# thilinarmtb/lsbench

Measured on AMD Instinct MI355X. Metric: cg_solves_per_sec, higher is better.
Workload: dtype f64

## Files before the change

### lsbench_amd/csrc/hip_kernels.hip

```cpp
#include "hip_kcommon.h"

__device__ __forceinline__ void spmv_publish(double *__restrict__ partials, double dot,
                                             double *sred, const lsb_ar_tail &tail) {
  if (!partials)
    return;
  double d[1] = {dot};
  wg_sum<1>(d, sred);
  if (tail.counter)
    ar_tail(partials, d[0], tail);
  else if (threadIdx.x == 0)
    partials[blockIdx.x] = d[0];
}

enum { SP_PREFETCH = 1, SP_NT = 2 };

template <int FLAGS, class T>
__device__ __forceinline__ T stream_load(const T *p) {
  if (FLAGS & SP_NT)
    return __builtin_nontemporal_load(p);
  return *p;
}

#define LSB_ISSUE_BLOCK(kk)                                                    \
  do {                                                                         \
// ... 722 lines not shown
      }
    } else if (row + 1 < n) {
      const sell_d2v o = {a0, a1};
      *(sell_d2v *)(y + row) = o;
      if (xdot) {
        dot = fma(a0, xd.x, dot);
        dot = fma(a1, xd.y, dot);
      }
    } else if (row < n) {
      y[row] = a0;
      if (xdot)
        dot = fma(a0, xd.x, dot);
    }
  }
#pragma unroll
  for (int k = 0; k < DEFER_DEPTH; k++)
    TMPL_UNPARK_SLOT(k);
#undef TMPL_UNPARK
#undef TMPL_UNPARK_SLOT
  if (stopped)
    return;
  spmv_publish(partials, dot, sred, tail);
}

template <int NF> struct col_ops {
  sell_d2u lo[NF > 1 ? NF - 1 : 1], hi[NF > 1 ? NF - 1 : 1];
  double edge;
  sell_d2v xd;
};
template <int NF> struct col_tmpl {
  int bc, bl[NF > 1 ? NF - 1 : 1], bh[NF > 1 ? NF - 1 : 1];
  double k0, kl[NF > 1 ? NF - 1 : 1], kc, kh[NF > 1 ? NF - 1 : 1], kL;
};
template <int NF, int DOT>
__device__ __forceinline__ void col_issue(col_ops<NF> &o, sell_d2u &cnext, const col_tmpl<NF> &T, const double *__restrict__ x,
                                          const double *__restrict__ xdot, long long gu, unsigned lrow, long long D,
                                          unsigned xlen, unsigned lane, bool with_next) {
  if (with_next)
    cnext = *(const sell_d2u *)(x + (gu + T.bc + D) + 2 * lane);
#pragma unroll
  for (int k = 0; k < NF - 1; k++) {
    o.lo[k] = *(const sell_d2u *)(x + (gu + T.bl[k]) + 2 * lane);
    o.hi[k] = *(const sell_d2u *)(x + (gu + T.bh[k]) + 2 * lane);
  }
  long long el = gu + T.bc - 1, er = gu + T.bc + (long long)LSB_SELL_ROWS;
  el = el < 0 ? 0 : el, er = er >= (long long)xlen ? (long long)xlen - 1 : er;
  o.edge = x[lane < 32u ? el : er];
  if (DOT == 2)
    o.xd = *(const sell_d2v *)(xdot + lrow + 2 * lane);
}
template <int NF, int DOT>
__device__ __forceinline__ void col_compute(const col_ops<NF> &o, const sell_d2u &cm, const sell_d2u &c, const sell_d2u &cp,
                                            const col_tmpl<NF> &T, double vm0, double vm1, double vp0, double vp1,
                                            unsigned lane, double &a0, double &a1, double &dot) {
  double up = lane_above(c.y), dn = lane_below(c.x);
  if (lane == 0)
    up = o.edge;
  if (lane == 63)
    dn = o.edge;
  a0 = fma(T.k0, cm.x, 0.0), a1 = fma(T.k0, cm.y, 0.0);
#pragma unroll
  for (int k = 0; k < NF - 1; k++)
    a0 = fma(T.kl[k], o.lo[k].x, a0), a1 = fma(T.kl[k], o.lo[k].y, a1);
  a0 = fma(vm0, vm0 != 0.0 ? up : 0.0, a0), a1 = fma(vm1, vm1 != 0.0 ? c.x : 0.0, a1);
  a0 = fma(T.kc, c.x, a0), a1 = fma(T.kc, c.y, a1);
  a0 = fma(vp0, vp0 != 0.0 ? c.y : 0.0, a0), a1 = fma(vp1, vp1 != 0.0 ? dn : 0.0, a1);
#pragma unroll
  for (int k = 0; k < NF - 1; k++)
    a0 = fma(T.kh[k], o.hi[k].x, a0), a1 = fma(T.kh[k], o.hi[k].y, a1);
  a0 = fma(T.kL, cp.x, a0), a1 = fma(T.kL, cp.y, a1);
  if (DOT == 1)
    dot = fma(a0, c.x, dot), dot = fma(a1, c.y, dot);
  else if (DOT == 2)
    dot = fma(a0, o.xd.x, dot), dot = fma(a1, o.xd.y, dot);
}

#define LSB_COL_HEAD 16
__device__ __forceinline__ bool col_walks_down(const unsigned *__restrict__ plan, unsigned dofs, unsigned it) {
  return dofs && ((plan[dofs + (it >> 5)] >> (it & 31u)) & 1u);
}
template <int NF, int DOT>
__global__ __launch_bounds__(WG, DOT == 2 ? 5 : 6) void k_spmv_tmpl_col(
    const unsigned *__restrict__ plan, unsigned period, unsigned n, unsigned row_begin, unsigned xlen,
    const unsigned *__restrict__ sptr, const unsigned long long *__restrict__ mask,
    const lsb_sell_tmpl *__restrict__ td, const int *__restrict__ sbase, const void *__restrict__ vals, int f32,
    const double *__restrict__ vconst, const double *__restrict__ x, double *__restrict__ y,
    const double *__restrict__ xdot, double *__restrict__ partials, const lsb_pcg_state *__restrict__ st,
    const lsb_ar_tail tail) {
  static_assert(NF >= 1 && NF <= 2, "one or two far slots per side");
  __shared__ double sred[4];
  const unsigned tid = threadIdx.x, lane = tid & 63u, wave = tid >> 6;
  const unsigned gx = gridDim.x / NXCD, xcd = blockIdx.x % NXCD, slot = blockIdx.x / NXCD;
  const unsigned i0 = plan[xcd], i1 = plan[xcd + 1];
  const u4v *__restrict__ items = (const u4v *)(plan + LSB_COL_HEAD);
  const unsigned dofs = plan[LSB_TMPL_COL_DOWN];
  const int stopped = st ? st->status : 0;
  const unsigned P = period * LSB_SELL_ROWS;
  double dot = 0.0;
  for (unsigned g = slot; i0 + 4 * g < i1; g += gx) {
    const unsigned it = __builtin_amdgcn_readfirstlane(i0 + 4 * g + wave);
    if (it >= i1)
      continue;
    const u4v rec = items[it];
    const unsigned s = __builtin_amdgcn_readfirstlane(rec.x), Kw = __builtin_amdgcn_readfirstlane(rec.y);
    const unsigned K = Kw & ~LSB_TMPL_COL_LOCKSTEP;
    const bool lockstep = (Kw & LSB_TMPL_COL_LOCKSTEP) != 0;
    if (K >= 2) {
      const unsigned t = __builtin_amdgcn_readfirstlane(rec.z), mb = __builtin_amdgcn_readfirstlane(rec.w);
      const lsb_sell_tmpl *T = td + t;
      col_tmpl<NF> C;
      C.bc = T->base[NF + 1];
      C.k0 = T->cst[0], C.kc = T->cst[NF + 1], C.kL = T->cst[2 * NF + 2];
// ... 75 lines not shown
          const sell_d2u v = *(const sell_d2u *)(x + (grow + r.x));
          a0 = fma(k, v.x, a0), a1 = fma(k, v.y, a1);
        } else {
          double v0, v1;
          if (f32) {
            const vt2<float>::type v = *((const vt2<float>::type *)((const float *)vals + (size_t)r.z * LSB_SELL_ROWS) + lane);
            v0 = (double)v.x, v1 = (double)v.y;
          } else {
            const sell_d2v v = *((const sell_d2v *)((const double *)vals + (size_t)r.z * LSB_SELL_ROWS) + lane);
            v0 = v.x, v1 = v.y;
          }
          const bool p0 = v0 != 0.0, p1 = v1 != 0.0;
          const double t0 = x[p0 ? grow + r.x : 0], t1 = x[p1 ? grow + 1 + r.x : 0];
          a0 = fma(v0, p0 ? t0 : 0.0, a0), a1 = fma(v1, p1 ? t1 : 0.0, a1);
        }
      }
      if (row + 1 < n) {
        const sell_d2v o = {a0, a1};
        *(sell_d2v *)(y + row) = o;
        if (DOT)
          dot = fma(a0, xd.x, dot), dot = fma(a1, xd.y, dot);
      } else if (row < n) {
        y[row] = a0;
        if (DOT)
          dot = fma(a0, xd.x, dot);
      }
    }
  }
  if (stopped)
    return;
  spmv_publish(partials, dot, sred, tail);
}

template <int NF> struct colp_c {
  sell_d2u rn, pn;
  sell_d2v xn, sn;
  double re, pe;
};
template <int NF> struct colp_m {
  sell_d2u rlo[NF > 1 ? NF - 1 : 1], plo[NF > 1 ? NF - 1 : 1], rhi[NF > 1 ? NF - 1 : 1], phi[NF > 1 ? NF - 1 : 1];
};
struct colp_out {
  sell_d2v q, x, p;
};
template <int NF, bool WITH_X, int NT>
__device__ __forceinline__ void colp_issue_c(colp_c<NF> &o, const col_tmpl<NF> &T, const double *__restrict__ r,
                                             const double *__restrict__ pold, const double *__restrict__ x,
                                             const double *pstale, long long gu, long long D, unsigned xlen,
                                             unsigned lane) {
  const long long ga = gu + T.bc + D;
  o.rn = *(const sell_d2u *)(r + ga + 2 * lane);
  o.pn = *(const sell_d2u *)(pold + ga + 2 * lane);
  if (WITH_X) {
    if (NT & 1) {
      o.xn = __builtin_nontemporal_load((const sell_d2v *)(x + (gu + D) + 2 * lane));
      o.sn = __builtin_nontemporal_load((const sell_d2v *)(pstale + (gu + D) + 2 * lane));
    } else {
      o.xn = *(const sell_d2v *)(x + (gu + D) + 2 * lane);
      o.sn = *(const sell_d2v *)(pstale + (gu + D) + 2 * lane);
    }
  }
  long long el = gu + T.bc - 1, er = gu + T.bc + (long long)LSB_SELL_ROWS;
  el = el < 0 ? 0 : el, er = er >= (long long)xlen ? (long long)xlen - 1 : er;
  const long long e = lane < 32u ? el : er;
  o.re = r[e], o.pe = pold[e];
}
template <int NF>
__device__ __forceinline__ void colp_issue_m(colp_m<NF> &o, const col_tmpl<NF> &T, const double *__restrict__ r,
                                             const double *__restrict__ pold, long long gu, unsigned lane) {
#pragma unroll
  for (int k = 0; k < NF - 1; k++) {
    o.rlo[k] = *(const sell_d2u *)(r + (gu + T.bl[k]) + 2 * lane);
    o.plo[k] = *(const sell_d2u *)(pold + (gu + T.bl[k]) + 2 * lane);
    o.rhi[k] = *(const sell_d2u *)(r + (gu + T.bh[k]) + 2 * lane);
    o.phi[k] = *(const sell_d2u *)(pold + (gu + T.bh[k]) + 2 * lane);
  }
}
template <int NF, bool OWNED, bool XUPD>
__device__ __forceinline__ void colp_compute(const colp_c<NF> &o, const colp_m<NF> &m, const sell_d2u &pb,
                                             const sell_d2u &p0, sell_d2u &pp, bool down, const col_tmpl<NF> &T, double vm0,
                                             double vm1, double vp0, double vp1, double beta, double alpha, double alpha2,
                                             double dc, unsigned lane, colp_out &out, double &dot) {
  pp.x = pnew_of(dc, o.rn.x, beta, o.pn.x), pp.y = pnew_of(dc, o.rn.y, beta, o.pn.y);
  if (OWNED) {
    if (XUPD) {
      out.x.x = (o.xn.x + alpha2 * o.sn.x) + alpha * o.pn.x, out.x.y = (o.xn.y + alpha2 * o.sn.y) + alpha * o.pn.y;
    }
    out.p.x = pp.x, out.p.y = pp.y;
  }
  const double edge = pnew_of(dc, o.re, beta, o.pe);
  double up = lane_above(p0.y), dn = lane_below(p0.x);
  if (lane == 0)
    up = edge;
  if (lane == 63)
    dn = edge;
  const sell_d2u &pm = down ? pp : pb, &pu = down ? pb : pp;
  double a0 = fma(T.k0, pm.x, 0.0), a1 = fma(T.k0, pm.y, 0.0);
#pragma unroll
  for (int k = 0; k < NF - 1; k++) {
    const double l0 = pnew_of(dc, m.rlo[k].x, beta, m.plo[k].x), l1 = pnew_of(dc, m.rlo[k].y, beta, m.plo[k].y);
    a0 = fma(T.kl[k], l0, a0), a1 = fma(T.kl[k], l1, a1);
  }
  a0 = fma(vm0, vm0 != 0.0 ? up : 0.0, a0), a1 = fma(vm1, vm1 != 0.0 ? p0.x : 0.0, a1);
  a0 = fma(T.kc, p0.x, a0), a1 = fma(T.kc, p0.y, a1);
  a0 = fma(vp0, vp0 != 0.0 ? p0.y : 0.0, a0), a1 = fma(vp1, vp1 != 0.0 ? dn : 0.0, a1);
#pragma unroll
  for (int k = 0; k < NF - 1; k++) {
    const double h0 = pnew_of(dc, m.rhi[k].x, beta, m.phi[k].x), h1 = pnew_of(dc, m.rhi[k].y, beta, m.phi[k].y);
// ... 20 lines not shown
  for (unsigned j = 0; j < len; j++) {
    const i4v rec = ((const i4v *)sbase)[q0 + j];
    if (rec.z < 0) {
      const double k = vconst[q0 + j];
      const sell_d2u rv = *(const sell_d2u *)(r + ((int)row + rec.x)), pv = *(const sell_d2u *)(pold + ((int)row + rec.x));
      a0 = fma(k, pnew_of(dc, rv.x, beta, pv.x), a0), a1 = fma(k, pnew_of(dc, rv.y, beta, pv.y), a1);
    } else {
      const sell_d2v v = *((const sell_d2v *)(vals + (size_t)rec.z * LSB_SELL_ROWS) + lane);
      const bool p0 = v.x != 0.0, p1 = v.y != 0.0;
      const int c0 = p0 ? (int)row + rec.x : 0, c1 = p1 ? (int)row + 1 + rec.x : 0;
      const double t0 = pnew_of(dc, r[c0], beta, pold[c0]), t1 = pnew_of(dc, r[c1], beta, pold[c1]);
      a0 = fma(v.x, p0 ? t0 : 0.0, a0), a1 = fma(v.y, p1 ? t1 : 0.0, a1);
    }
  }
  const double n0 = pnew_of(dc, r0, beta, o0), n1 = pnew_of(dc, r1, beta, o1);
  if (l0) {
    pnew[row] = n0;
    if (xupd)
      x[row] = (x0 + alpha2 * s0) + alpha * o0;
    if (q)
      q[row] = a0;
    dot = fma(a0, n0, dot);
  }
  if (l1) {
    pnew[row + 1] = n1;
    if (xupd)
      x[row + 1] = (x1 + alpha2 * s1) + alpha * o1;
    if (q)
      q[row + 1] = a1;
    dot = fma(a1, n1, dot);
  }
}

#define COLP_ST(PTR, V, BIT)                                                                   \
  do {                                                                                         \
    if (NT & (BIT))                                                                            \
      __builtin_nontemporal_store((V), (sell_d2v *)(PTR));                                     \
    else                                                                                       \
      *(sell_d2v *)(PTR) = (V);                                                                \
  } while (0)
#define COLP_STORE(OUT, LROW, WITH_Q, WITH_XP)                                                 \
  do {                                                                                         \
    if (WITH_Q)                                                                                \
      COLP_ST(q + (LROW) + 2 * lane, (OUT).q, 2);                                              \
    if (WITH_XP) {                                                                             \
      if (XUPD)                                                                                \
        COLP_ST(x + ((LROW) + Du) + 2 * lane, (OUT).x, 1);                                     \
      COLP_ST(pnew + ((LROW) + Du) + 2 * lane, (OUT).p, 2);                                    \
    }                                                                                          \
  } while (0)

template <int NF, int NT, bool XUPD>
__global__ __launch_bounds__(WG, NF == 2 ? 3 : 5) void k_pcg_col_px(
    const unsigned *__restrict__ plan, unsigned period, unsigned n, const unsigned *__restrict__ sptr,
    const unsigned long long *__restrict__ mask, const lsb_sell_tmpl *__restrict__ td, const int *__restrict__ sbase,
    const double *__restrict__ vals, const double *__restrict__ vconst, const double *__restrict__ r,
    const double *__restrict__ pold, double *pnew, double *__restrict__ x, double dc,
    double *__restrict__ partials, lsb_pcg_state *__restrict__ st, int parity,
    const double *__restrict__ parts2, unsigned nparts2) {
  static_assert(NF >= 1 && NF <= 2, "one or two far slots per side");
  __shared__ double sred[8];
  double *const q = nullptr;
  const unsigned tid = threadIdx.x, lane = tid & 63u, wave = tid >> 6;
  const unsigned gx = gridDim.x / NXCD, xcd = blockIdx.x % NXCD, slot = blockIdx.x / NXCD;
  const int stopped = st->status;
  const double rz_old = st->rz[parity], thresh2 = st->thresh2, alpha = st->alpha[0], alpha2 = st->alpha[1];
  const unsigned i0 = plan[xcd], i1 = plan[xcd + 1];
  double v[2];
  wg_sum_partials<2>(parts2, nparts2, v, sred);
  if (stopped)
    return;
  const double rz_new = v[0], rr = v[1];
  const bool conv = rr <= thresh2;
  if (blockIdx.x == 0 && threadIdx.x == 0) {
    const int it = st->iters + 1;
    st->iters = it;
    st->rr = rr;
    st->rz[parity ^ 1] = rz_new;
    if (conv)
      st->status = LSB_STATUS_CONVERGED;
    else {
      if (XUPD)
        st->xpend = 0;
      if (it >= st->maxit)
        st->pad = 1;
    }
  }
  if (conv)
    return;
  const double beta = rz_new / rz_old;
  const u4v *__restrict__ items = (const u4v *)(plan + LSB_COL_HEAD);
  const unsigned dofs = plan[LSB_TMPL_COL_DOWN];
  const unsigned P = period * LSB_SELL_ROWS;
  double dot = 0.0;
  for (unsigned g = slot; i0 + 4 * g < i1; g += gx) {
    const unsigned it = __builtin_amdgcn_readfirstlane(i0 + 4 * g + wave);
    if (it >= i1)
      continue;
    const u4v rec = items[it];
    const unsigned s = __builtin_amdgcn_readfirstlane(rec.x);
    const unsigned K = __builtin_amdgcn_readfirstlane(rec.y) & ~LSB_TMPL_COL_LOCKSTEP;
    if (K >= 3) {
      const unsigned t = __builtin_amdgcn_readfirstlane(rec.z), mb = __builtin_amdgcn_readfirstlane(rec.w);
      const lsb_sell_tmpl *T = td + t;
      col_tmpl<NF> C;
      C.bc = T->base[NF + 1];
      C.k0 = T->cst[0], C.kc = T->cst[NF + 1], C.kL = T->cst[2 * NF + 2];
#pragma unroll
      for (int k = 0; k < NF - 1; k++) {
        C.bl[k] = T->base[1 + k], C.bh[k] = T->base[NF + 3 + k];
        C.kl[k] = T->cst[1 + k], C.kh[k] = T->cst[NF + 3 + k];
      }
      const int side_k[2] = {T->kidx[NF], T->kidx[NF + 2]}, side_kd[2] = {T->kind[NF], T->kind[NF + 2]};
      const bool down = col_walks_down(plan, dofs, it);
      const unsigned s0 = down ? s + (K - 1) * period : s;
      const long long D = down ? -(long long)P : (long long)P;
      const unsigned Du = (unsigned)D;
      long long gu = (long long)s0 * LSB_SELL_ROWS;
      unsigned lrow = s0 * LSB_SELL_ROWS;
      const long long gc = gu + C.bc;
      const sell_d2u rb = *(const sell_d2u *)(r + (gc - D) + 2 * lane);
      const sell_d2u pb = *(const sell_d2u *)(pold + (gc - D) + 2 * lane);
      const sell_d2u r0 = *(const sell_d2u *)(r + gc + 2 * lane), o0 = *(const sell_d2u *)(pold + gc + 2 * lane);
      sell_d2v x0 = {0.0, 0.0}, s0v = {0.0, 0.0};
      if (XUPD)
        x0 = *(const sell_d2v *)(x + lrow + 2 * lane), s0v = *(const sell_d2v *)(pnew + lrow + 2 * lane);
      colp_c<NF> c0, c1;
      colp_m<NF> m0, m1, m2;
      colp_issue_c<NF, XUPD, NT>(c0, C, r, pold, x, pnew, gu, D, n, lane);
      colp_issue_m<NF>(m0, C, r, pold, gu, lane);
      colp_issue_m<NF>(m1, C, r, pold, gu + D, lane);
      unsigned long long mk[2][2] = {{0ull, 0ull}, {0ull, 0ull}};
#pragma unroll
      for (int side = 0; side < 2; side++)
        if (side_k[side] >= 0 && side_kd[side] == 2) {
          const unsigned long long *mp = mask + 2 * ((size_t)mb + (unsigned)side_k[side]);
          mk[side][0] = mp[0], mk[side][1] = mp[1];
        }
      double vm0 = T->cst[NF], vm1 = vm0, vp0 = T->cst[NF + 2], vp1 = vp0;
      if (side_k[0] >= 0 || side_k[1] >= 0)
        tmpl_side_values(T, NF, 0u, lane, side_k, side_kd, mk, vals, 0, vm0, vm1, vp0, vp1);
      sell_d2u pm, p0, pp;
      pm.x = pnew_of(dc, rb.x, beta, pb.x), pm.y = pnew_of(dc, rb.y, beta, pb.y);
      p0.x = pnew_of(dc, r0.x, beta, o0.x), p0.y = pnew_of(dc, r0.y, beta, o0.y);
      colp_out res;
      res.x.x = (x0.x + alpha2 * s0v.x) + alpha * o0.x, res.x.y = (x0.y + alpha2 * s0v.y) + alpha * o0.y;
      res.p.x = p0.x, res.p.y = p0.y;
      res.q = res.p;
      COLP_STORE(res, lrow - Du, false, true);
      for (unsigned k = 0; k + 2 < K; k++) {
        colp_issue_c<NF, XUPD, NT>(c1, C, r, pold, x, pnew, gu + D, D, n, lane);
        colp_issue_m<NF>(m2, C, r, pold, gu + 2 * D, lane);
        colp_compute<NF, true, XUPD>(c0, m0, pm, p0, pp, down, C, vm0, vm1, vp0, vp1, beta, alpha, alpha2, dc, lane, res, dot);
        COLP_STORE(res, lrow, false, true);
        pm = p0, p0 = pp, c0 = c1, m0 = m1, m1 = m2;
        gu += D, lrow += Du;
      }
      colp_issue_c<NF, false, NT>(c1, C, r, pold, x, pnew, gu + D, D, n, lane);
      colp_compute<NF, true, XUPD>(c0, m0, pm, p0, pp, down, C, vm0, vm1, vp0, vp1, beta, alpha, alpha2, dc, lane, res, dot);
      COLP_STORE(res, lrow, false, true);
      pm = p0, p0 = pp, c0 = c1, m0 = m1;
      gu += D, lrow += Du;
      colp_compute<NF, false, XUPD>(c0, m0, pm, p0, pp, down, C, vm0, vm1, vp0, vp1, beta, alpha, alpha2, dc, lane, res, dot);
      COLP_STORE(res, lrow, false, false);
    } else {
      for (unsigned k = 0; k < K; k++)
        colp_single(s + k * period, n, lane, sptr, sbase, vals, vconst, r, pold, pnew, x, nullptr, beta, alpha, alpha2,
                    XUPD, dc, dot);
    }
  }
  if (partials) {
    double d[1] = {dot};
    wg_sum<1>(d, sred);
    if (threadIdx.x == 0)
      partials[blockIdx.x] = d[0];
  }
}
#undef COLP_STORE
#undef COLP_ST

template <int NF>
__global__ __launch_bounds__(WG, 5) void k_pcg_col_r(
    const unsigned *__restrict__ plan, unsigned period, unsigned n, const unsigned *__restrict__ sptr,
    const unsigned long long *__restrict__ mask, const lsb_sell_tmpl *__restrict__ td, const int *__restrict__ sbase,
    const double *__restrict__ vals, const double *__restrict__ vconst, const double *__restrict__ p,
    double *__restrict__ r, double dc, lsb_pcg_state *__restrict__ st, int parity, int pbuf, int xtwo,
    const double *__restrict__ pq_parts, unsigned npq, double *__restrict__ partials2) {
  static_assert(NF >= 1 && NF <= 2, "one or two far slots per side");
  __shared__ double sred[8];
  const unsigned tid = threadIdx.x, lane = tid & 63u, wave = tid >> 6;
  const unsigned gx = gridDim.x / NXCD, xcd = blockIdx.x % NXCD, slot = blockIdx.x / NXCD;
  const int stopped = st->status, pad = st->pad;
  const double rz = st->rz[parity];
  const unsigned i0 = plan[xcd], i1 = plan[xcd + 1];
  double pqv[1];
  wg_sum_partials<1>(pq_parts, npq, pqv, sred);
  if (stopped)
    return;
  if (pad) {
    if (blockIdx.x == 0 && threadIdx.x == 0)
      st->status = LSB_STATUS_MAXIT;
    return;
  }
  const double pq = pqv[0];
  if (!(pq != 0.0) || !isfinite(pq)) {
    if (blockIdx.x == 0 && threadIdx.x == 0)
      st->status = LSB_STATUS_BREAKDOWN;
    return;
  }
  const double alpha = rz / pq;
  if (blockIdx.x == 0 && threadIdx.x == 0) {
    st->pq = pq, st->alpha[1] = st->alpha[0], st->alpha[0] = alpha, st->xpend = (xtwo ? 3 : 1) + pbuf;
  }
  const u4v *__restrict__ items = (const u4v *)(plan + LSB_COL_HEAD);
  const unsigned dofs = plan[LSB_TMPL_COL_DOWN];
  const unsigned P = period * LSB_SELL_ROWS;
  double acc[2] = {0.0, 0.0}, nodot = 0.0;
#define COLR_FINISH(A0, A1, RV, LROW)                                                          \
  do {                                                                                         \
    sell_d2v rn_;                                                                              \
    rn_.x = (RV).x - alpha * (A0), rn_.y = (RV).y - alpha * (A1);                              \
    *(sell_d2v *)(r + (LROW) + 2 * lane) = rn_;                                                \
    acc[0] += rn_.x * (dc * rn_.x);                                                            \
    acc[0] += rn_.y * (dc * rn_.y);                                                            \
    acc[1] += rn_.x * rn_.x;                                                                   \
    acc[1] += rn_.y * rn_.y;                                                                   \
  } while (0)
  for (unsigned g = slot; i0 + 4 * g < i1; g += gx) {
    const unsigned it = __builtin_amdgcn_readfirstlane(i0 + 4 * g + wave);
    if (it >= i1)
      continue;
    const u4v rec = items[it];
    const unsigned s = __builtin_amdgcn_readfirstlane(rec.x);
    const unsigned K = __builtin_amdgcn_readfirstlane(rec.y) & ~LSB_TMPL_COL_LOCKSTEP;
    if (K >= 3) {
      const unsigned t = __builtin_amdgcn_readfirstlane(rec.z), mb = __builtin_amdgcn_readfirstlane(rec.w);
      const lsb_sell_tmpl *T = td + t;
      col_tmpl<NF> C;
      C.bc = T->base[NF + 1];
      C.k0 = T->cst[0], C.kc = T->cst[NF + 1], C.kL = T->cst[2 * NF + 2];
#pragma unroll
      for (int k = 0; k < NF - 1; k++) {
        C.bl[k] = T->base[1 + k], C.bh[k] = T->base[NF + 3 + k];
        C.kl[k] = T->cst[1 + k], C.kh[k] = T->cst[NF + 3 + k];
      }
      const int side_k[2] = {T->kidx[NF], T->kidx[NF + 2]}, side_kd[2] = {T->kind[NF], T->kind[NF + 2]};
      const bool down = col_walks_down(plan, dofs, it);
      const unsigned s0 = down ? s + (K - 1) * period : s;
      const long long D = down ? -(long long)P : (long long)P;
      const unsigned Du = (unsigned)D;
      long long gu = (long long)s0 * LSB_SELL_ROWS;
      unsigned lrow = s0 * LSB_SELL_ROWS;
      col_ops<NF> cur, nxt;
      sell_d2u cb = *(const sell_d2u *)(p + (gu + C.bc - D) + 2 * lane);
      sell_d2u c0 = *(const sell_d2u *)(p + (gu + C.bc) + 2 * lane);
      sell_d2u ca, cn;
      col_issue<NF, 2>(cur, ca, C, p, r, gu, lrow, D, n, lane, true);
      unsigned long long mk[2][2] = {{0ull, 0ull}, {0ull, 0ull}};
#pragma unroll
      for (int side = 0; side < 2; side++)
        if (side_k[side] >= 0 && side_kd[side] == 2) {
          const unsigned long long *mp = mask + 2 * ((size_t)mb + (unsigned)side_k[side]);
          mk[side][0] = mp[0], mk[side][1] = mp[1];
        }
      double vm0 = T->cst[NF], vm1 = vm0, vp0 = T->cst[NF + 2], vp1 = vp0;
      if (side_k[0] >= 0 || side_k[1] >= 0)
        tmpl_side_values(T, NF, 0u, lane, side_k, side_kd, mk, vals, 0, vm0, vm1, vp0, vp1);
      for (unsigned k = 0; k + 1 < K; k++) {
        col_issue<NF, 2>(nxt, cn, C, p, r, gu + D, lrow + Du, D, n, lane, true);
        double a0, a1;
        col_compute<NF, 0>(cur, down ? ca : cb, c0, down ? cb : ca, C, vm0, vm1, vp0, vp1, lane, a0, a1, nodot);
        COLR_FINISH(a0, a1, cur.xd, lrow);
        cb = c0, c0 = ca, ca = cn, cur = nxt;
        gu += D, lrow += Du;
      }
      double a0, a1;
      col_compute<NF, 0>(cur, down ? ca : cb, c0, down ? cb : ca, C, vm0, vm1, vp0, vp1, lane, a0, a1, nodot);
      COLR_FINISH(a0, a1, cur.xd, lrow);
    } else {
      for (unsigned k = 0; k < K; k++) {
        const unsigned sl = s + k * period, row = sl * LSB_SELL_ROWS + 2 * lane;
        const unsigned q0 = sptr[sl] / LSB_SELL_ROWS, len = (sptr[sl + 1] - sptr[sl]) / LSB_SELL_ROWS;
        const bool l0 = row < n, l1 = row + 1 < n;
        const double r0 = l0 ? r[row] : 0.0, r1 = l1 ? r[row + 1] : 0.0;
        double a0 = 0.0, a1 = 0.0;
        for (unsigned j = 0; j < len; j++) {
          const i4v rec2 = ((const i4v *)sbase)[q0 + j];
          if (rec2.z < 0) {
            const double kk = vconst[q0 + j];
            const sell_d2u pv = *(const sell_d2u *)(p + ((int)row + rec2.x));
            a0 = fma(kk, pv.x, a0), a1 = fma(kk, pv.y, a1);
          } else {
            const sell_d2v v = *((const sell_d2v *)(vals + (size_t)rec2.z * LSB_SELL_ROWS) + lane);
            const bool p0 = v.x != 0.0, p1 = v.y != 0.0;
            const double t0 = p[p0 ? (int)row + rec2.x : 0], t1 = p[p1 ? (int)row + 1 + rec2.x : 0];
            a0 = fma(v.x, p0 ? t0 : 0.0, a0), a1 = fma(v.y, p1 ? t1 : 0.0, a1);
          }
        }
        if (l0) {
          const double rn0 = r0 - alpha * a0;
          r[row] = rn0;
          acc[0] += rn0 * (dc * rn0), acc[1] += rn0 * rn0;
        }
        if (l1) {
          const double rn1 = r1 - alpha * a1;
          r[row + 1] = rn1;
          acc[0] += rn1 * (dc * rn1), acc[1] += rn1 * rn1;
        }
      }
    }
  }
#undef COLR_FINISH
  wg_sum<2>(acc, sred);
  if (threadIdx.x == 0) {
    partials2[2 * blockIdx.x + 0] = acc[0];
    partials2[2 * blockIdx.x + 1] = acc[1];
  }
}


__device__ __forceinline__ unsigned bin_pad(unsigned i) { return i + (i >> 3); }

template <int FLAGS, int BIN_U>
__global__ __launch_bounds__(WG) void k_spmv_binned(
    const unsigned *__restrict__ chunk_begin, unsigned nchunk, const unsigned *__restrict__ rows,
    const unsigned *__restrict__ cols, const double *__restrict__ vals,
    const double *__restrict__ x, double *__restrict__ y, const lsb_pcg_state *__restrict__ st) {
  constexpr unsigned CHUNK = BIN_U * WG;
  __shared__ double sprod[CHUNK + CHUNK / 8 + 8];
  __shared__ unsigned skey[CHUNK + CHUNK / 8 + 8];
  __shared__ double swv[4];
  __shared__ int swf[4];
  __shared__ double sred[4];
  const unsigned tid = threadIdx.x, lane = tid & 63u, wave = tid >> 6;
  const unsigned per = gridDim.x / NXCD;
  const unsigned w = (blockIdx.x % NXCD) * per + blockIdx.x / NXCD;
  if (w >= nchunk)
    return;
  const unsigned e0 = chunk_begin[w], cnt = chunk_begin[w + 1] - e0;
  unsigned r[BIN_U], c[BIN_U];
  double v[BIN_U];
  if (cnt <= CHUNK) {
#pragma unroll
// ... 375 lines not shown
```

### lsbench_amd/csrc/lsb_operator.c

```c
#include "lsb_impl.h"
#include <string.h>
#ifdef _OPENMP
#include <omp.h>
#else
static inline int omp_get_max_threads(void) { return 1; }
#endif

static struct csr *csr_alloc(unsigned nrows, unsigned long long nnz) {
  if (nnz > 0xFFFFFFFFull)
    errx(EXIT_FAILURE, "CSR with %llu non-zeros does not fit 32-bit offsets "
                       "(reference layout, src/lsbench-impl.h:22-26)", nnz);
  struct csr *S = lsb_calloc(struct csr, 1);
  S->nrows = nrows, S->base = 0;
  S->offs = lsb_calloc(unsigned, (size_t)nrows + 1);
  S->cols = lsb_calloc(unsigned, (size_t)nnz);
  S->vals = lsb_calloc(double, (size_t)nnz);
  if (!S->offs || !S->cols || !S->vals)
    errx(EXIT_FAILURE, "out of host memory for a %u-row / %llu-nnz CSR", nrows, nnz);
  return S;
}

void lsb_csr_free(struct csr *A) {
  if (!A)
    return;
// ... 1422 lines not shown
    CC_FAIL(13, "walk directions on z-groups of %u cells, %u items per XCD and turn", period, LSB_TMPL_COL_TURN(T->nfar));
  seen = (unsigned char *)calloc((size_t)ns + 1, 1);
  if (!seen)
    CC_FAIL(4, "out of memory");
  const unsigned nplanes = (ns + period - 1) / period, ngroups = (nplanes + C->kmax - 1) / C->kmax;
  for (unsigned i = 0; i < C->nitem; i++) {
    const unsigned *it = C->item + 4 * (size_t)i;
    const unsigned s = it[0], run = it[1] & ~LSB_TMPL_COL_LOCKSTEP;
    if (it[1] & LSB_TMPL_COL_LOCKSTEP) {
      unsigned xk = 0;
      while (xk + 1 < LSB_COL_XCDS && C->xbeg[xk + 1] <= i)
        xk++;
      const unsigned g0 = C->xbeg[xk] + (i - C->xbeg[xk]) / 4 * 4;
      if (g0 + 4 > C->xbeg[xk + 1])
        CC_FAIL(12, "item %u: lockstep in a turn of fewer than four items", i);
      for (unsigned w = 0; w < 4; w++)
        if (C->item[4 * (size_t)(g0 + w) + 1] != it[1] || run < 2)
          CC_FAIL(12, "item %u: lockstep, but item %u of its turn has another length", i, g0 + w);
    }
    if (run < 1 || run > C->kmax || s < C->s_lo || (unsigned long long)s + (unsigned long long)(run - 1) * period >= C->s_hi)
      CC_FAIL(5, "item %u: %u slices from slice %u, every %u, of [%u, %u)", i, run, s, period, C->s_lo, C->s_hi);
    for (unsigned k = 0; k < run; k++) {
      const unsigned sk = s + k * period;
      if (seen[sk]++)
        CC_FAIL(6, "item %u: slice %u is in two items", i, sk);
      if (run >= 2 && (!col_member(T, sk, period) || !col_same(T, s, sk)))
        CC_FAIL(7, "item %u: slice %u does not continue the column of slice %u", i, sk, s);
    }
    if (run >= 2 && C->centre0 && T->t[T->tid[s]].base[T->nfar + 1] != 0)
      CC_FAIL(10, "item %u: centre base %d in a plan that says 0", i, T->t[T->tid[s]].base[T->nfar + 1]);
    if (run >= 2 && (it[2] != T->tid[s] || it[3] != T->vbase[2 * (size_t)s + 1]))
      CC_FAIL(8, "item %u: template %u / first mask %u, its first slice has %u / %u", i, it[2], it[3], T->tid[s],
              T->vbase[2 * (size_t)s + 1]);
    if (C->down) {
      const unsigned zg = (unsigned)(((unsigned long long)(s / period + 1) * ngroups - 1) / nplanes);
      if (((C->down[i / 32] >> (i % 32)) & 1u) != ((zg & 1u) && run >= 3))
        CC_FAIL(13, "item %u: %u slices walk %s in z-group %u", i, run, ((zg & 1u) && run >= 3) ? "upward" : "downward", zg);
    }
  }
  for (unsigned s = C->s_lo; s < C->s_hi; s++)
    if (!seen[s])
      CC_FAIL(9, "slice %u is in no item", s);
  free(seen);
  return 0;
#undef CC_FAIL
}

void lsb_tmpl_cols_free(struct lsb_tmpl_cols *C) {
  if (!C)
    return;
  free(C->item), free(C->down), free(C);
}

void lsb_sell_tmpls_free(struct lsb_sell_tmpls *T) {
  if (!T)
    return;
  free(T->tid), free(T->vbase), free(T->mask), free(T->t), free(T);
}

void lsb_sell_vc_free(struct lsb_sell_vc *V) {
  if (!V)
    return;
  free(V->slots), free(V->vconst), free(V->vals), free(V);
}

void lsb_sell_free(struct lsb_sell *S) {
// ... 5 lines not shown
```

Measured before the change: 1.085.

## Prefetch next column item's header and first loads during current item tail

The column-walk PCG kernels (k_pcg_col_p and k_pcg_col_r) now load the next work item's plan record, template constants and first-slice operands while the current item's last slices are still being computed. The first item's loads are also issued before the partial-sum reduction. This hides the load latency at item boundaries. The side-value computation is simplified to a mask-only path, and a host-side plan check is added that rejects templates where that simplification would be wrong. Several loads and stores also get wave-uniform base pointers through readfirstlane casts into the global address space, to allow scalar addressing. The cost is higher register pressure from carrying the next item's state, which could hurt occupancy under the existing launch bounds.

After: 1.098, median of 6. About the same (+1.1%).

```diff
diff --git a/lsbench_amd/csrc/hip_kernels.hip b/lsbench_amd/csrc/hip_kernels.hip
--- a/lsbench_amd/csrc/hip_kernels.hip
+++ b/lsbench_amd/csrc/hip_kernels.hip
@@ -778,17 +778,21 @@
   int bc, bl[NF > 1 ? NF - 1 : 1], bh[NF > 1 ? NF - 1 : 1];
   double k0, kl[NF > 1 ? NF - 1 : 1], kc, kh[NF > 1 ? NF - 1 : 1], kL;
 };
-template <int NF, int DOT>
+template <int NF, int DOT, int PART = 3>
 __device__ __forceinline__ void col_issue(col_ops<NF> &o, sell_d2u &cnext, const col_tmpl<NF> &T, const double *__restrict__ x,
                                           const double *__restrict__ xdot, long long gu, unsigned lrow, long long D,
                                           unsigned xlen, unsigned lane, bool with_next) {
-  if (with_next)
+  if ((PART & 1) && with_next)
     cnext = *(const sell_d2u *)(x + (gu + T.bc + D) + 2 * lane);
-#pragma unroll
-  for (int k = 0; k < NF - 1; k++) {
-    o.lo[k] = *(const sell_d2u *)(x + (gu + T.bl[k]) + 2 * lane);
-    o.hi[k] = *(const sell_d2u *)(x + (gu + T.bh[k]) + 2 * lane);
-  }
+  if (PART & 2) {
+#pragma unroll
+    for (int k = 0; k < NF - 1; k++) {
+      o.lo[k] = *(const sell_d2u *)(x + (gu + T.bl[k]) + 2 * lane);
+      o.hi[k] = *(const sell_d2u *)(x + (gu + T.bh[k]) + 2 * lane);
+    }
+  }
+  if (!(PART & 1))
+    return;
   long long el = gu + T.bc - 1, er = gu + T.bc + (long long)LSB_SELL_ROWS;
   el = el < 0 ? 0 : el, er = er >= (long long)xlen ? (long long)xlen - 1 : er;
   o.edge = x[lane < 32u ? el : er];
@@ -824,6 +828,70 @@
 #define LSB_COL_HEAD 16
 __device__ __forceinline__ bool col_walks_down(const unsigned *__restrict__ plan, unsigned dofs, unsigned it) {
   return dofs && ((plan[dofs + (it >> 5)] >> (it & 31u)) & 1u);
+}
+template <int NF> struct col_head {
+  unsigned s, K;
+  unsigned t, mb;
+  unsigned down;
+  unsigned masked;
+  col_tmpl<NF> C;
+  double cm, cp;
+  unsigned long long mk[2][2];
+};
+template <int NF>
+__device__ __forceinline__ void col_head_none(col_head<NF> &H) {
+  H.s = 0, H.K = 0, H.t = 0, H.mb = 0, H.down = 0;
+}
+template <int NF>
+__device__ __forceinline__ void col_head_load(col_head<NF> &H, const unsigned *__restrict__ plan, unsigned dofs, unsigned it,
+                                              const lsb_sell_tmpl *__restrict__ td) {
+  const u4v rec = ((const u4v *)(plan + LSB_COL_HEAD))[it];
+  H.s = __builtin_amdgcn_readfirstlane(rec.x);
+  H.K = __builtin_amdgcn_readfirstlane(rec.y) & ~LSB_TMPL_COL_LOCKSTEP;
+  H.t = __builtin_amdgcn_readfirstlane(rec.z), H.mb = __builtin_amdgcn_readfirstlane(rec.w);
+  H.down = 0;
+  if (H.K >= 3) {
+    const lsb_sell_tmpl *T = td + H.t;
+    H.C.bc = T->base[NF + 1];
+    H.down = col_walks_down(plan, dofs, it) ? 1u : 0u;
+  }
+}
+template <int NF>
+__device__ __forceinline__ void col_head_consts(col_head<NF> &H, const lsb_sell_tmpl *__restrict__ td,
+                                                const unsigned long long *__restrict__ mask) {
+  const lsb_sell_tmpl *T = td + H.t;
+  H.C.k0 = T->cst[0], H.C.kc = T->cst[NF + 1], H.C.kL = T->cst[2 * NF + 2];
+#pragma unroll
+  for (int k = 0; k < NF - 1; k++) {
+    H.C.bl[k] = T->base[1 + k], H.C.bh[k] = T->base[NF + 3 + k];
+    H.C.kl[k] = T->cst[1 + k], H.C.kh[k] = T->cst[NF + 3 + k];
+  }
+  H.cm = T->cst[NF], H.cp = T->cst[NF + 2];
+  H.masked = 0;
+#pragma unroll
+  for (int side = 0; side < 2; side++) {
+    const int k = T->kidx[NF + 2 * side], kd = T->kind[NF + 2 * side];
+    H.mk[side][0] = 0ull, H.mk[side][1] = 0ull;
+    if (k >= 0 && kd == 2) {
+      const unsigned long long *mp = mask + 2 * ((size_t)H.mb + (unsigned)k);
+      H.mk[side][0] = mp[0], H.mk[side][1] = mp[1];
+      H.masked |= 1u << side;
+    }
+  }
+}
+template <int NF>
+__device__ __forceinline__ void col_head_sides(const col_head<NF> &H, unsigned lane, double &vm0, double &vm1, double &vp0,
+                                               double &vp1) {
+  const unsigned sh = (2u * lane) & 63u;
+  vm0 = vm1 = H.cm, vp0 = vp1 = H.cp;
+  if (H.masked & 1u) {
+    const unsigned long long w = (lane & 32u) ? H.mk[0][1] : H.mk[0][0];
+    vm0 = (w >> sh) & 1ull ? H.cm : 0.0, vm1 = (w >> (sh + 1u)) & 1ull ? H.cm : 0.0;
+  }
+  if (H.masked & 2u) {
+    const unsigned long long w = (lane & 32u) ? H.mk[1][1] : H.mk[1][0];
+    vp0 = (w >> sh) & 1ull ? H.cp : 0.0, vp1 = (w >> (sh + 1u)) & 1ull ? H.cp : 0.0;
+  }
 }
 template <int NF, int DOT>
 __global__ __launch_bounds__(WG, DOT == 2 ? 5 : 6) void k_spmv_tmpl_col(
@@ -965,6 +1033,12 @@
   spmv_publish(partials, dot, sred, tail);
 }
 
+#define COL_G __attribute__((address_space(1)))
+__device__ __forceinline__ const COL_G double *col_uni(const double *p) {
+  const unsigned long long v = (unsigned long long)p;
+  const unsigned lo = __builtin_amdgcn_readfirstlane((unsigned)v), hi = __builtin_amdgcn_readfirstlane((unsigned)(v >> 32));
+  return (const COL_G double *)(((unsigned long long)hi << 32) | lo);
+}
 template <int NF> struct colp_c {
   sell_d2u rn, pn;
   sell_d2v xn, sn;
@@ -976,37 +1050,41 @@
 struct colp_out {
   sell_d2v q, x, p;
 };
+template <int NF, int NT>
+__device__ __forceinline__ void colp_issue_x(colp_c<NF> &o, const double *x, const double *pstale, long long gu, long long D,
+                                             unsigned lane) {
+  if (NT & 1) {
+    o.xn = __builtin_nontemporal_load((const COL_G sell_d2v *)(col_uni(x + (gu + D)) + 2 * lane));
+    o.sn = __builtin_nontemporal_load((const COL_G sell_d2v *)(col_uni(pstale + (gu + D)) + 2 * lane));
+  } else {
+    o.xn = *(const COL_G sell_d2v *)(col_uni(x + (gu + D)) + 2 * lane);
+    o.sn = *(const COL_G sell_d2v *)(col_uni(pstale + (gu + D)) + 2 * lane);
+  }
+}
 template <int NF, bool WITH_X, int NT>
 __device__ __forceinline__ void colp_issue_c(colp_c<NF> &o, const col_tmpl<NF> &T, const double *__restrict__ r,
                                              const double *__restrict__ pold, const double *__restrict__ x,
                                              const double *pstale, long long gu, long long D, unsigned xlen,
                                              unsigned lane) {
   const long long ga = gu + T.bc + D;
-  o.rn = *(const sell_d2u *)(r + ga + 2 * lane);
-  o.pn = *(const sell_d2u *)(pold + ga + 2 * lane);
-  if (WITH_X) {
-    if (NT & 1) {
-      o.xn = __builtin_nontemporal_load((const sell_d2v *)(x + (gu + D) + 2 * lane));
-      o.sn = __builtin_nontemporal_load((const sell_d2v *)(pstale + (gu + D) + 2 * lane));
-    } else {
-      o.xn = *(const sell_d2v *)(x + (gu + D) + 2 * lane);
-      o.sn = *(const sell_d2v *)(pstale + (gu + D) + 2 * lane);
-    }
-  }
+  o.rn = *(const COL_G sell_d2u *)(col_uni(r + ga) + 2 * lane);
+  o.pn = *(const COL_G sell_d2u *)(col_uni(pold + ga) + 2 * lane);
+  if (WITH_X)
+    colp_issue_x<NF, NT>(o, x, pstale, gu, D, lane);
   long long el = gu + T.bc - 1, er = gu + T.bc + (long long)LSB_SELL_ROWS;
   el = el < 0 ? 0 : el, er = er >= (long long)xlen ? (long long)xlen - 1 : er;
-  const long long e = lane < 32u ? el : er;
-  o.re = r[e], o.pe = pold[e];
+  const unsigned eo = lane < 32u ? 0u : (unsigned)(er - el);
+  o.re = col_uni(r + el)[eo], o.pe = col_uni(pold + el)[eo];
 }
 template <int NF>
 __device__ __forceinline__ void colp_issue_m(colp_m<NF> &o, const col_tmpl<NF> &T, const double *__restrict__ r,
                                              const double *__restrict__ pold, long long gu, unsigned lane) {
 #pragma unroll
   for (int k = 0; k < NF - 1; k++) {
-    o.rlo[k] = *(const sell_d2u *)(r + (gu + T.bl[k]) + 2 * lane);
-    o.plo[k] = *(const sell_d2u *)(pold + (gu + T.bl[k]) + 2 * lane);
-    o.rhi[k] = *(const sell_d2u *)(r + (gu + T.bh[k]) + 2 * lane);
-    o.phi[k] = *(const sell_d2u *)(pold + (gu + T.bh[k]) + 2 * lane);
+    o.rlo[k] = *(const COL_G sell_d2u *)(col_uni(r + (gu + T.bl[k])) + 2 * lane);
+    o.plo[k] = *(const COL_G sell_d2u *)(col_uni(pold + (gu + T.bl[k])) + 2 * lane);
+    o.rhi[k] = *(const COL_G sell_d2u *)(col_uni(r + (gu + T.bh[k])) + 2 * lane);
+    o.phi[k] = *(const COL_G sell_d2u *)(col_uni(pold + (gu + T.bh[k])) + 2 * lane);
   }
 }
 template <int NF, bool OWNED, bool XUPD>
@@ -1093,12 +1171,29 @@
   }
 }
 
+template <int NF> struct colp_first {
+  sell_d2u rb, pb, r0, o0;
+  colp_c<NF> c0;
+};
+template <int NF, int NT>
+__device__ __forceinline__ void colp_first_issue(colp_first<NF> &F, const col_head<NF> &H, unsigned period,
+                                                 const double *__restrict__ r, const double *__restrict__ pold,
+                                                 unsigned n, unsigned lane) {
+  const unsigned s0 = H.down ? H.s + (H.K - 1) * period : H.s;
+  const long long P = (long long)period * LSB_SELL_ROWS, D = H.down ? -P : P;
+  const long long gu = (long long)s0 * LSB_SELL_ROWS, gc = gu + H.C.bc;
+  F.rb = *(const COL_G sell_d2u *)(col_uni(r + (gc - D)) + 2 * lane);
+  F.pb = *(const COL_G sell_d2u *)(col_uni(pold + (gc - D)) + 2 * lane);
+  F.r0 = *(const COL_G sell_d2u *)(col_uni(r + gc) + 2 * lane), F.o0 = *(const COL_G sell_d2u *)(col_uni(pold + gc) + 2 * lane);
+  colp_issue_c<NF, false, NT>(F.c0, H.C, r, pold, nullptr, nullptr, gu, D, n, lane);
+}
+
 #define COLP_ST(PTR, V, BIT)                                                                   \
   do {                                                                                         \
     if (NT & (BIT))                                                                            \
-      __builtin_nontemporal_store((V), (sell_d2v *)(PTR));                                     \
+      __builtin_nontemporal_store((V), (COL_G sell_d2v *)(PTR));                               \
     else                                                                                       \
-      *(sell_d2v *)(PTR) = (V);                                                                \
+      *(COL_G sell_d2v *)(PTR) = (V);                                                          \
   } while (0)
 #define COLP_STORE(OUT, LROW, WITH_Q, WITH_XP)                                                 \
   do {                                                                                         \
@@ -1106,8 +1201,8 @@
       COLP_ST(q + (LROW) + 2 * lane, (OUT).q, 2);                                              \
     if (WITH_XP) {                                                                             \
       if (XUPD)                                                                                \
-        COLP_ST(x + ((LROW) + Du) + 2 * lane, (OUT).x, 1);                                     \
-      COLP_ST(pnew + ((LROW) + Du) + 2 * lane, (OUT).p, 2);                                    \
+        COLP_ST((COL_G double *)col_uni(x + ((LROW) + Du)) + 2 * lane, (OUT).x, 1);                  \
+      COLP_ST((COL_G double *)col_uni(pnew + ((LROW) + Du)) + 2 * lane, (OUT).p, 2);                 \
     }                                                                                          \
   } while (0)
 
@@ -1127,6 +1222,18 @@
   const int stopped = st->status;
   const double rz_old = st->rz[parity], thresh2 = st->thresh2, alpha = st->alpha[0], alpha2 = st->alpha[1];
   const unsigned i0 = plan[xcd], i1 = plan[xcd + 1];
+  const unsigned dofs = plan[LSB_TMPL_COL_DOWN];
+  const unsigned it0 = __builtin_amdgcn_readfirstlane(i0 + 4 * slot + wave);
+  col_head<NF> H;
+  colp_first<NF> F;
+  col_head_none(H);
+  if (it0 < i1) {
+    col_head_load(H, plan, dofs, it0, td);
+    if (H.K >= 3) {
+      colp_first_issue<NF, NT>(F, H, period, r, pold, n, lane);
+      col_head_consts(H, td, mask);
+    }
+  }
   double v[2];
   wg_sum_partials<2>(parts2, nparts2, v, sred);
   if (stopped)
@@ -1150,62 +1257,38 @@
   if (conv)
     return;
   const double beta = rz_new / rz_old;
-  const u4v *__restrict__ items = (const u4v *)(plan + LSB_COL_HEAD);
-  const unsigned dofs = plan[LSB_TMPL_COL_DOWN];
   const unsigned P = period * LSB_SELL_ROWS;
   double dot = 0.0;
-  for (unsigned g = slot; i0 + 4 * g < i1; g += gx) {
-    const unsigned it = __builtin_amdgcn_readfirstlane(i0 + 4 * g + wave);
-    if (it >= i1)
-      continue;
-    const u4v rec = items[it];
-    const unsigned s = __builtin_amdgcn_readfirstlane(rec.x);
-    const unsigned K = __builtin_amdgcn_readfirstlane(rec.y) & ~LSB_TMPL_COL_LOCKSTEP;
-    if (K >= 3) {
-      const unsigned t = __builtin_amdgcn_readfirstlane(rec.z), mb = __builtin_amdgcn_readfirstlane(rec.w);
-      const lsb_sell_tmpl *T = td + t;
-      col_tmpl<NF> C;
-      C.bc = T->base[NF + 1];
-      C.k0 = T->cst[0], C.kc = T->cst[NF + 1], C.kL = T->cst[2 * NF + 2];
-#pragma unroll
-      for (int k = 0; k < NF - 1; k++) {
-        C.bl[k] = T->base[1 + k], C.bh[k] = T->base[NF + 3 + k];
-        C.kl[k] = T->cst[1 + k], C.kh[k] = T->cst[NF + 3 + k];
-      }
-      const int side_k[2] = {T->kidx[NF], T->kidx[NF + 2]}, side_kd[2] = {T->kind[NF], T->kind[NF + 2]};
-      const bool down = col_walks_down(plan, dofs, it);
-      const unsigned s0 = down ? s + (K - 1) * period : s;
+  for (unsigned it = it0; it < i1;) {
+    const unsigned itn = __builtin_amdgcn_readfirstlane(it + 4 * gx);
+    col_head<NF> Hn;
+    colp_first<NF> Fn = {};
+    col_head_none(Hn);
+    if (H.K >= 3) {
+      const unsigned K = H.K;
+      const col_tmpl<NF> C = H.C;
+      const bool down = H.down != 0;
+      const unsigned s0 = down ? H.s + (K - 1) * period : H.s;
       const long long D = down ? -(long long)P : (long long)P;
       const unsigned Du = (unsigned)D;
       long long gu = (long long)s0 * LSB_SELL_ROWS;
       unsigned lrow = s0 * LSB_SELL_ROWS;
-      const long long gc = gu + C.bc;
-      const sell_d2u rb = *(const sell_d2u *)(r + (gc - D) + 2 * lane);
-      const sell_d2u pb = *(const sell_d2u *)(pold + (gc - D) + 2 * lane);
-      const sell_d2u r0 = *(const sell_d2u *)(r + gc + 2 * lane), o0 = *(const sell_d2u *)(pold + gc + 2 * lane);
+      colp_c<NF> c0 = F.c0, c1;
+      colp_m<NF> m0, m1, m2;
       sell_d2v x0 = {0.0, 0.0}, s0v = {0.0, 0.0};
-      if (XUPD)
-        x0 = *(const sell_d2v *)(x + lrow + 2 * lane), s0v = *(const sell_d2v *)(pnew + lrow + 2 * lane);
-      colp_c<NF> c0, c1;
-      colp_m<NF> m0, m1, m2;
-      colp_issue_c<NF, XUPD, NT>(c0, C, r, pold, x, pnew, gu, D, n, lane);
+      if (XUPD) {
+        x0 = *(const COL_G sell_d2v *)(col_uni(x + lrow) + 2 * lane), s0v = *(const COL_G sell_d2v *)(col_uni(pnew + lrow) + 2 * lane);
+        colp_issue_x<NF, NT>(c0, x, pnew, gu, D, lane);
+      }
       colp_issue_m<NF>(m0, C, r, pold, gu, lane);
       colp_issue_m<NF>(m1, C, r, pold, gu + D, lane);
-      unsigned long long mk[2][2] = {{0ull, 0ull}, {0ull, 0ull}};
-#pragma unroll
-      for (int side = 0; side < 2; side++)
-        if (side_k[side] >= 0 && side_kd[side] == 2) {
-          const unsigned long long *mp = mask + 2 * ((size_t)mb + (unsigned)side_k[side]);
-          mk[side][0] = mp[0], mk[side][1] = mp[1];
-        }
-      double vm0 = T->cst[NF], vm1 = vm0, vp0 = T->cst[NF + 2], vp1 = vp0;
-      if (side_k[0] >= 0 || side_k[1] >= 0)
-        tmpl_side_values(T, NF, 0u, lane, side_k, side_kd, mk, vals, 0, vm0, vm1, vp0, vp1);
+      double vm0, vm1, vp0, vp1;
+      col_head_sides(H, lane, vm0, vm1, vp0, vp1);
       sell_d2u pm, p0, pp;
-      pm.x = pnew_of(dc, rb.x, beta, pb.x), pm.y = pnew_of(dc, rb.y, beta, pb.y);
-      p0.x = pnew_of(dc, r0.x, beta, o0.x), p0.y = pnew_of(dc, r0.y, beta, o0.y);
+      pm.x = pnew_of(dc, F.rb.x, beta, F.pb.x), pm.y = pnew_of(dc, F.rb.y, beta, F.pb.y);
+      p0.x = pnew_of(dc, F.r0.x, beta, F.o0.x), p0.y = pnew_of(dc, F.r0.y, beta, F.o0.y);
       colp_out res;
-      res.x.x = (x0.x + alpha2 * s0v.x) + alpha * o0.x, res.x.y = (x0.y + alpha2 * s0v.y) + alpha * o0.y;
+      res.x.x = (x0.x + alpha2 * s0v.x) + alpha * F.o0.x, res.x.y = (x0.y + alpha2 * s0v.y) + alpha * F.o0.y;
       res.p.x = p0.x, res.p.y = p0.y;
       res.q = res.p;
       COLP_STORE(res, lrow - Du, false, true);
@@ -1218,17 +1301,34 @@
         gu += D, lrow += Du;
       }
       colp_issue_c<NF, false, NT>(c1, C, r, pold, x, pnew, gu + D, D, n, lane);
+      if (itn < i1)
+        col_head_load(Hn, plan, dofs, itn, td);
       colp_compute<NF, true, XUPD>(c0, m0, pm, p0, pp, down, C, vm0, vm1, vp0, vp1, beta, alpha, alpha2, dc, lane, res, dot);
       COLP_STORE(res, lrow, false, true);
       pm = p0, p0 = pp, c0 = c1, m0 = m1;
       gu += D, lrow += Du;
-      colp_compute<NF, false, XUPD>(c0, m0, pm, p0, pp, down, C, vm0, vm1, vp0, vp1, beta, alpha, alpha2, dc, lane, res, dot);
-      COLP_STORE(res, lrow, false, false);
+      if (Hn.K >= 3) {
+        colp_first_issue<NF, NT>(Fn, Hn, period, r, pold, n, lane);
+        colp_compute<NF, false, XUPD>(c0, m0, pm, p0, pp, down, C, vm0, vm1, vp0, vp1, beta, alpha, alpha2, dc, lane, res, dot);
+        COLP_STORE(res, lrow, false, false);
+      } else {
+        colp_compute<NF, false, XUPD>(c0, m0, pm, p0, pp, down, C, vm0, vm1, vp0, vp1, beta, alpha, alpha2, dc, lane, res, dot);
+        COLP_STORE(res, lrow, false, false);
+      }
     } else {
-      for (unsigned k = 0; k < K; k++)
-        colp_single(s + k * period, n, lane, sptr, sbase, vals, vconst, r, pold, pnew, x, nullptr, beta, alpha, alpha2,
+      for (unsigned k = 0; k < H.K; k++)
+        colp_single(H.s + k * period, n, lane, sptr, sbase, vals, vconst, r, pold, pnew, x, nullptr, beta, alpha, alpha2,
                     XUPD, dc, dot);
-    }
+      if (itn < i1) {
+        col_head_load(Hn, plan, dofs, itn, td);
+        if (Hn.K >= 3)
+          colp_first_issue<NF, NT>(Fn, Hn, period, r, pold, n, lane);
+      }
+    }
+    H = Hn, F = Fn;
+    if (H.K >= 3)
+      col_head_consts(H, td, mask);
+    it = itn;
   }
   if (partials) {
     double d[1] = {dot};
@@ -1240,6 +1340,21 @@
 #undef COLP_STORE
 #undef COLP_ST
 
+template <int NF> struct colr_first {
+  sell_d2u cb, c0, ca;
+  col_ops<NF> cur;
+};
+template <int NF>
+__device__ __forceinline__ void colr_first_issue(colr_first<NF> &F, const col_head<NF> &H, unsigned period,
+                                                 const double *__restrict__ p, const double *r, unsigned n,
+                                                 unsigned lane) {
+  const unsigned s0 = H.down ? H.s + (H.K - 1) * period : H.s;
+  const long long P = (long long)period * LSB_SELL_ROWS, D = H.down ? -P : P;
+  const long long gu = (long long)s0 * LSB_SELL_ROWS;
+  F.cb = *(const sell_d2u *)(p + (gu + H.C.bc - D) + 2 * lane);
+  F.c0 = *(const sell_d2u *)(p + (gu + H.C.bc) + 2 * lane);
+  col_issue<NF, 2, 1>(F.cur, F.ca, H.C, p, r, gu, s0 * LSB_SELL_ROWS, D, n, lane, true);
+}
 template <int NF>
 __global__ __launch_bounds__(WG, 5) void k_pcg_col_r(
     const unsigned *__restrict__ plan, unsigned period, unsigned n, const unsigned *__restrict__ sptr,
@@ -1254,6 +1369,18 @@
   const int stopped = st->status, pad = st->pad;
   const double rz = st->rz[parity];
   const unsigned i0 = plan[xcd], i1 = plan[xcd + 1];
+  const unsigned dofs = plan[LSB_TMPL_COL_DOWN];
+  const unsigned it0 = __builtin_amdgcn_readfirstlane(i0 + 4 * slot + wave);
+  col_head<NF> H;
+  colr_first<NF> F;
+  col_head_none(H);
+  if (it0 < i1) {
+    col_head_load(H, plan, dofs, it0, td);
+    if (H.K >= 3) {
+      colr_first_issue<NF>(F, H, period, p, r, n, lane);
+      col_head_consts(H, td, mask);
+    }
+  }
   double pqv[1];
   wg_sum_partials<1>(pq_parts, npq, pqv, sred);
   if (stopped)
@@ -1273,8 +1400,6 @@
   if (blockIdx.x == 0 && threadIdx.x == 0) {
     st->pq = pq, st->alpha[1] = st->alpha[0], st->alpha[0] = alpha, st->xpend = (xtwo ? 3 : 1) + pbuf;
   }
-  const u4v *__restrict__ items = (const u4v *)(plan + LSB_COL_HEAD);
-  const unsigned dofs = plan[LSB_TMPL_COL_DOWN];
   const unsigned P = period * LSB_SELL_ROWS;
   double acc[2] = {0.0, 0.0}, nodot = 0.0;
 #define COLR_FINISH(A0, A1, RV, LROW)                                                          \
@@ -1287,57 +1412,48 @@
     acc[1] += rn_.x * rn_.x;                                                                   \
     acc[1] += rn_.y * rn_.y;                                                                   \
   } while (0)
-  for (unsigned g = slot; i0 + 4 * g < i1; g += gx) {
-    const unsigned it = __builtin_amdgcn_readfirstlane(i0 + 4 * g + wave);
-    if (it >= i1)
-      continue;
-    const u4v rec = items[it];
-    const unsigned s = __builtin_amdgcn_readfirstlane(rec.x);
-    const unsigned K = __builtin_amdgcn_readfirstlane(rec.y) & ~LSB_TMPL_COL_LOCKSTEP;
+  for (unsigned it = it0; it < i1;) {
+    const unsigned itn = __builtin_amdgcn_readfirstlane(it + 4 * gx);
+    col_head<NF> Hn;
+    colr_first<NF> Fn = {};
+    col_head_none(Hn);
+    const unsigned s = H.s, K = H.K;
     if (K >= 3) {
-      const unsigned t = __builtin_amdgcn_readfirstlane(rec.z), mb = __builtin_amdgcn_readfirstlane(rec.w);
-      const lsb_sell_tmpl *T = td + t;
-      col_tmpl<NF> C;
-      C.bc = T->base[NF + 1];
-      C.k0 = T->cst[0], C.kc = T->cst[NF + 1], C.kL = T->cst[2 * NF + 2];
-#pragma unroll
-      for (int k = 0; k < NF - 1; k++) {
-        C.bl[k] = T->base[1 + k], C.bh[k] = T->base[NF + 3 + k];
-        C.kl[k] = T->cst[1 + k], C.kh[k] = T->cst[NF + 3 + k];
-      }
-      const int side_k[2] = {T->kidx[NF], T->kidx[NF + 2]}, side_kd[2] = {T->kind[NF], T->kind[NF + 2]};
-      const bool down = col_walks_down(plan, dofs, it);
+      const col_tmpl<NF> C = H.C;
+      const bool down = H.down != 0;
       const unsigned s0 = down ? s + (K - 1) * period : s;
       const long long D = down ? -(long long)P : (long long)P;
       const unsigned Du = (unsigned)D;
       long long gu = (long long)s0 * LSB_SELL_ROWS;
       unsigned lrow = s0 * LSB_SELL_ROWS;
-      col_ops<NF> cur, nxt;
-      sell_d2u cb = *(const sell_d2u *)(p + (gu + C.bc - D) + 2 * lane);
-      sell_d2u c0 = *(const sell_d2u *)(p + (gu + C.bc) + 2 * lane);
-      sell_d2u ca, cn;
-      col_issue<NF, 2>(cur, ca, C, p, r, gu, lrow, D, n, lane, true);
-      unsigned long long mk[2][2] = {{0ull, 0ull}, {0ull, 0ull}};
-#pragma unroll
-      for (int side = 0; side < 2; side++)
-        if (side_k[side] >= 0 && side_kd[side] == 2) {
-          const unsigned long long *mp = mask + 2 * ((size_t)mb + (unsigned)side_k[side]);
-          mk[side][0] = mp[0], mk[side][1] = mp[1];
-        }
-      double vm0 = T->cst[NF], vm1 = vm0, vp0 = T->cst[NF + 2], vp1 = vp0;
-      if (side_k[0] >= 0 || side_k[1] >= 0)
-        tmpl_side_values(T, NF, 0u, lane, side_k, side_kd, mk, vals, 0, vm0, vm1, vp0, vp1);
-      for (unsigned k = 0; k + 1 < K; k++) {
+      col_ops<NF> cur = F.cur, nxt;
+      sell_d2u cb = F.cb, c0 = F.c0, ca = F.ca, cn;
+      col_issue<NF, 2, 2>(cur, ca, C, p, r, gu, lrow, D, n, lane, true);
+      double vm0, vm1, vp0, vp1;
+      col_head_sides(H, lane, vm0, vm1, vp0, vp1);
+      double a0, a1;
+      for (unsigned k = 0; k + 2 < K; k++) {
         col_issue<NF, 2>(nxt, cn, C, p, r, gu + D, lrow + Du, D, n, lane, true);
-        double a0, a1;
         col_compute<NF, 0>(cur, down ? ca : cb, c0, down ? cb : ca, C, vm0, vm1, vp0, vp1, lane, a0, a1, nodot);
         COLR_FINISH(a0, a1, cur.xd, lrow);
         cb = c0, c0 = ca, ca = cn, cur = nxt;
         gu += D, lrow += Du;
       }
-      double a0, a1;
+      col_issue<NF, 2>(nxt, cn, C, p, r, gu + D, lrow + Du, D, n, lane, true);
+      if (itn < i1)
+        col_head_load(Hn, plan, dofs, itn, td);
       col_compute<NF, 0>(cur, down ? ca : cb, c0, down ? cb : ca, C, vm0, vm1, vp0, vp1, lane, a0, a1, nodot);
       COLR_FINISH(a0, a1, cur.xd, lrow);
+      cb = c0, c0 = ca, ca = cn, cur = nxt;
+      gu += D, lrow += Du;
+      if (Hn.K >= 3) {
+        colr_first_issue<NF>(Fn, Hn, period, p, r, n, lane);
+        col_compute<NF, 0>(cur, down ? ca : cb, c0, down ? cb : ca, C, vm0, vm1, vp0, vp1, lane, a0, a1, nodot);
+        COLR_FINISH(a0, a1, cur.xd, lrow);
+      } else {
+        col_compute<NF, 0>(cur, down ? ca : cb, c0, down ? cb : ca, C, vm0, vm1, vp0, vp1, lane, a0, a1, nodot);
+        COLR_FINISH(a0, a1, cur.xd, lrow);
+      }
     } else {
       for (unsigned k = 0; k < K; k++) {
         const unsigned sl = s + k * period, row = sl * LSB_SELL_ROWS + 2 * lane;
@@ -1369,7 +1485,16 @@
           acc[0] += rn1 * (dc * rn1), acc[1] += rn1 * rn1;
         }
       }
-    }
+      if (itn < i1) {
+        col_head_load(Hn, plan, dofs, itn, td);
+        if (Hn.K >= 3)
+          colr_first_issue<NF>(Fn, Hn, period, p, r, n, lane);
+      }
+    }
+    H = Hn, F = Fn;
+    if (H.K >= 3)
+      col_head_consts(H, td, mask);
+    it = itn;
   }
 #undef COLR_FINISH
   wg_sum<2>(acc, sred);
diff --git a/lsbench_amd/csrc/lsb_operator.c b/lsbench_amd/csrc/lsb_operator.c
--- a/lsbench_amd/csrc/lsb_operator.c
+++ b/lsbench_amd/csrc/lsb_operator.c
@@ -1478,6 +1478,17 @@
     if (run >= 2 && (it[2] != T->tid[s] || it[3] != T->vbase[2 * (size_t)s + 1]))
       CC_FAIL(8, "item %u: template %u / first mask %u, its first slice has %u / %u", i, it[2], it[3], T->tid[s],
               T->vbase[2 * (size_t)s + 1]);
+    if (run >= 3) {
+      if (it[2] >= T->ntmpl)
+        CC_FAIL(14, "item %u: asked for ahead, but its template %u is none of the layout's %u", i, it[2], T->ntmpl);
+      const struct lsb_sell_tmpl *t = &T->t[it[2]];
+      for (int side = 0; side < 2; side++) {
+        const int j = (int)T->nfar + 2 * side;
+        if (t->kidx[j] >= 0 && (t->kind[j] != 2 || (unsigned long long)it[3] + (unsigned)t->kidx[j] >= T->nmask))
+          CC_FAIL(14, "item %u: asked for ahead, but slot %d of its template is kind %d, mask %u + %d of %llu", i, j,
+                  t->kind[j], it[3], t->kidx[j], T->nmask);
+      }
+    }
     if (C->down) {
       const unsigned zg = (unsigned)(((unsigned long long)(s / period + 1) * ngroups - 1) / nplanes);
       if (((C->down[i / 32] >> (i % 32)) & 1u) != ((zg & 1u) && run >= 3))
```
